# MikeIvanichev/norma

Measured on AMD Instinct MI355X. Metric: audio-sec/wall-sec (xRT) distil-large-v3 fp16 b32, higher is better.
Workload: dtype f16

## Files before the change

### norma_amd/csrc/k_attn_enc.hip

```cpp
#include "nh_kernels.h"

#ifndef ENC_ATTN_KERNEL
#define ENC_ATTN_KERNEL enc_attn_kernel
#define ENC_ATTN_LAUNCH launch_enc_attention
#endif
#define KT 64
#define QW 32
#ifndef ENC_ATTN_WAVES
#define ENC_ATTN_WAVES 8
#endif
#define QB (QW * ENC_ATTN_WAVES)
#define NTHR (64 * ENC_ATTN_WAVES)
#define NSLOT (NTHR >= 512 ? 1 : 512 / NTHR)
#define TILE_B 8192

__device__ __forceinline__ int swap23(int x) { return (x & ~12) | ((x & 4) << 1) | ((x & 8) >> 1); }

#ifndef ENC_ATTN_MINWAVES
#ifdef ENC_ATTN_PIPE
#define ENC_ATTN_MINWAVES 2
#else
#define ENC_ATTN_MINWAVES 4
#endif
#endif
__global__ __launch_bounds__(NTHR, (NTHR <= 512 ? ENC_ATTN_MINWAVES : 1)) void ENC_ATTN_KERNEL(const half_t *__restrict__ q, const half_t *__restrict__ k,
                                                         long ld, const half_t *__restrict__ vt,
                                                         half_t *__restrict__ out, long ldo, int S, int H) {
    __shared__ __attribute__((aligned(16))) char smem[2 * 2 * TILE_B];
    const int tid = threadIdx.x, lane = tid & 63, w = tid >> 6;
    const int r = lane & 31, hh = lane >> 5;
    const int b = blockIdx.z, h = blockIdx.y;
    const int q0 = blockIdx.x * QB + w * QW;
    const int nT = (S + KT - 1) / KT;

    half8 qf[4];
    {
        int qrow = q0 + r; if (qrow >= S) qrow = S - 1;
        const half_t *qp = q + ((long)b * S + qrow) * ld + h * NH_DH + 8 * hh;
#pragma unroll
        for (int ks = 0; ks < 4; ks++) qf[ks] = *reinterpret_cast<const half8 *>(qp + 16 * ks);
    }
    const half_t *kg[NSLOT]; const half_t *vg[NSLOT];
    int krow_off[NSLOT];
#pragma unroll
    for (int i = 0; i < NSLOT; i++) {
        int row = (tid >> 3) + (NTHR / 8) * i;
        int c = (tid & 7) ^ ((row >> 1) & 7);
        krow_off[i] = swap23(row);
        kg[i] = k + (long)b * S * ld + h * NH_DH + c * 8;
        vg[i] = vt + ((long)(b * H + h) * NH_DH + row) * NH_SP + c * 8;
    }
    u32x4 rk[NSLOT], rv[NSLOT];
    const bool stager = NTHR <= 512 || tid < 512;
    auto load_k = [&](int t) {
        if (!stager) return;
#pragma unroll
        for (int i = 0; i < NSLOT; i++) {
            int key = t * KT + krow_off[i]; if (key >= S) key = S - 1;
            rk[i] = *reinterpret_cast<const u32x4 *>(kg[i] + (long)key * ld);
        }
    };
    auto load_v = [&](int t) {
        if (!stager) return;
#pragma unroll
        for (int i = 0; i < NSLOT; i++) rv[i] = *reinterpret_cast<const u32x4 *>(vg[i] + t * KT);
    };
    auto store_k = [&](int buf) {
        if (!stager) return;
        u32x4 *lk = reinterpret_cast<u32x4 *>(smem + buf * 2 * TILE_B);
#pragma unroll
        for (int i = 0; i < NSLOT; i++) lk[tid + NTHR * i] = rk[i];
    };
    auto store_v = [&](int buf) {
        if (!stager) return;
        u32x4 *lv = reinterpret_cast<u32x4 *>(smem + buf * 2 * TILE_B + TILE_B);
#pragma unroll
        for (int i = 0; i < NSLOT; i++) lv[tid + NTHR * i] = rv[i];
    };
    auto load_tile = [&](int t) { load_k(t); load_v(t); };
    auto store_tile = [&](int buf) { store_k(buf); store_v(buf); };
    load_tile(0);
    store_tile(0);
#ifdef ENC_ATTN_PIPE
    if (nT > 1) { load_k(1); store_k(1); }
#endif
    __syncthreads();

    const int g = (r >> 1) & 7;
    const int offK0 = r * 128 + ((hh ^ g) << 4);
    const int offV0 = r * 128 + ((hh ^ g) << 4);

    f32x16 o0, o1;
#pragma unroll
    for (int i = 0; i < 16; i++) { o0[i] = 0.f; o1[i] = 0.f; }
    const f32x16 zero = {0.f, 0.f, 0.f, 0.f, 0.f, 0.f, 0.f, 0.f, 0.f, 0.f, 0.f, 0.f, 0.f, 0.f, 0.f, 0.f};
    const half_t one_h = hh == 0 ? (half_t)1.0f : (half_t)0.0f;
    const half8 kx = {one_h, one_h, (half_t)0.f, (half_t)0.f, (half_t)0.f, (half_t)0.f, (half_t)0.f, (half_t)0.f};
    half8 qx = {(half_t)0.f, (half_t)0.f, (half_t)0.f, (half_t)0.f, (half_t)0.f, (half_t)0.f, (half_t)0.f, (half_t)0.f};
    float m_ref = 0.f, l_run = 0.f;
    const float REBASE = 8.0f;

    f32x16 s0, s1;
    auto qk_phase = [&](const char *tk, f32x16 &s0, f32x16 &s1) {
        {
            half8 k0 = *reinterpret_cast<const half8 *>(tk + offK0);
            half8 k1 = *reinterpret_cast<const half8 *>(tk + 4096 + offK0);
            s0 = __builtin_amdgcn_mfma_f32_32x32x16_f16(k0, qf[0], zero, 0, 0, 0);
            s1 = __builtin_amdgcn_mfma_f32_32x32x16_f16(k1, qf[0], zero, 0, 0, 0);
        }
#pragma unroll
        for (int ks = 1; ks < 4; ks++) {
            half8 k0 = *reinterpret_cast<const half8 *>(tk + (offK0 ^ (ks << 5)));
            half8 k1 = *reinterpret_cast<const half8 *>(tk + 4096 + (offK0 ^ (ks << 5)));
            s0 = __builtin_amdgcn_mfma_f32_32x32x16_f16(k0, qf[ks], s0, 0, 0, 0);
            s1 = __builtin_amdgcn_mfma_f32_32x32x16_f16(k1, qf[ks], s1, 0, 0, 0);
        }
        s0 = __builtin_amdgcn_mfma_f32_32x32x16_f16(kx, qx, s0, 0, 0, 0);
        s1 = __builtin_amdgcn_mfma_f32_32x32x16_f16(kx, qx, s1, 0, 0, 0);
    };
    auto sm_head = [&](int t) {
        if (t * KT + KT > S) {
#pragma unroll
            for (int i = 0; i < 16; i++) {
                int rho = (i & 3) + 8 * (i >> 2) + 4 * hh;
                int key0 = t * KT + swap23(rho), key1 = t * KT + 32 + swap23(rho);
                if (key0 >= S) s0[i] = -INFINITY;
                if (key1 >= S) s1[i] = -INFINITY;
            }
        }
        float mx = fmaxf(fmaxf(s0[0], s0[1]), s0[2]);
#pragma unroll
        for (int i = 3; i < 15; i += 2) mx = fmaxf(fmaxf(mx, s0[i]), s0[i + 1]);
        mx = fmaxf(fmaxf(mx, s0[15]), s1[0]);
#pragma unroll
        for (int i = 1; i < 15; i += 2) mx = fmaxf(fmaxf(mx, s1[i]), s1[i + 1]);
        mx = fmaxf(mx, s1[15]);
        mx = fmaxf(mx, __shfl_xor(mx, 32));
        const bool reb = (t == 0) || (mx > REBASE);
        if (__builtin_amdgcn_ballot_w64(reb) != 0) {
            const float dlt = reb ? mx : 0.f;
            const float alpha = __builtin_amdgcn_exp2f(-dlt);
#pragma unroll
            for (int i = 0; i < 16; i++) { o0[i] *= alpha; o1[i] *= alpha; s0[i] -= dlt; s1[i] -= dlt; }
            l_run *= alpha;
            m_ref += dlt;
            const float nm = fminf(fmaxf(-m_ref, -60000.f), 60000.f);
            const half_t hi = (half_t)nm;
            const half_t lo = (half_t)(nm - (float)hi);
            qx[0] = hh == 0 ? hi : (half_t)0.f;
            qx[1] = hh == 0 ? lo : (half_t)0.f;
        }
    };
    auto sm_body = [&](const char *tv) {
        float ps = 0.f;
#pragma unroll
        for (int i = 0; i < 16; i++) {
            s0[i] = __builtin_amdgcn_exp2f(s0[i]); s1[i] = __builtin_amdgcn_exp2f(s1[i]);
            ps += s0[i]; ps += s1[i];
        }
        l_run += ps;
        half8 p00, p01, p10, p11;
#pragma unroll
        for (int j = 0; j < 8; j++) {
            p00[j] = (half_t)s0[j]; p01[j] = (half_t)s0[8 + j];
            p10[j] = (half_t)s1[j]; p11[j] = (half_t)s1[8 + j];
        }
        {
            half8 v;
            v = *reinterpret_cast<const half8 *>(tv + (offV0 ^ (0 << 4)));          o0 = __builtin_amdgcn_mfma_f32_32x32x16_f16(v, p00, o0, 0, 0, 0);
            v = *reinterpret_cast<const half8 *>(tv + 4096 + (offV0 ^ (0 << 4)));   o1 = __builtin_amdgcn_mfma_f32_32x32x16_f16(v, p00, o1, 0, 0, 0);
            v = *reinterpret_cast<const half8 *>(tv + (offV0 ^ (2 << 4)));          o0 = __builtin_amdgcn_mfma_f32_32x32x16_f16(v, p01, o0, 0, 0, 0);
            v = *reinterpret_cast<const half8 *>(tv + 4096 + (offV0 ^ (2 << 4)));   o1 = __builtin_amdgcn_mfma_f32_32x32x16_f16(v, p01, o1, 0, 0, 0);
            v = *reinterpret_cast<const half8 *>(tv + (offV0 ^ (4 << 4)));          o0 = __builtin_amdgcn_mfma_f32_32x32x16_f16(v, p10, o0, 0, 0, 0);
            v = *reinterpret_cast<const half8 *>(tv + 4096 + (offV0 ^ (4 << 4)));   o1 = __builtin_amdgcn_mfma_f32_32x32x16_f16(v, p10, o1, 0, 0, 0);
            v = *reinterpret_cast<const half8 *>(tv + (offV0 ^ (6 << 4)));          o0 = __builtin_amdgcn_mfma_f32_32x32x16_f16(v, p11, o0, 0, 0, 0);
            v = *reinterpret_cast<const half8 *>(tv + 4096 + (offV0 ^ (6 << 4)));   o1 = __builtin_amdgcn_mfma_f32_32x32x16_f16(v, p11, o1, 0, 0, 0);
        }
    };
#ifndef ENC_ATTN_PIPE
    int cur = 0;
    for (int t = 0; t < nT; t++) {
        const bool more = (t + 1 < nT);
        if (more) load_tile(t + 1);
        qk_phase(smem + cur * 2 * TILE_B, s0, s1);
        sm_head(t);
        sm_body(smem + cur * 2 * TILE_B + TILE_B);
        if (more) store_tile(cur ^ 1);
        __syncthreads();
        cur ^= 1;
    }
#else
    f32x16 n0, n1;
    qk_phase(smem, s0, s1);
    for (int t = 0; t < nT; t++) {
        if (t + 2 < nT) load_k(t + 2);
        if (t + 1 < nT) load_v(t + 1);
        sm_head(t);
        qk_phase(smem + ((t + 1) & 1) * 2 * TILE_B, n0, n1);
        sm_body(smem + (t & 1) * 2 * TILE_B + TILE_B);
#pragma unroll
        for (int i = 0; i < 18; i++) {
            __builtin_amdgcn_sched_group_barrier(0x008, 1, 0);
            __builtin_amdgcn_sched_group_barrier(0x002, ENC_ATTN_PIPE, 0);
        }
        if (t + 2 < nT) store_k(t & 1);
        if (t + 1 < nT) store_v((t + 1) & 1);
        __syncthreads();
        s0 = n0; s1 = n1;
    }
#endif
    const float l_tot = l_run + __shfl_xor(l_run, 32);
    const float inv = 1.0f / l_tot;
    const int qrow = q0 + r;
    if (qrow < S) {
        half_t *op = out + ((long)b * S + qrow) * ldo + h * NH_DH + 4 * hh;
#pragma unroll
        for (int gq = 0; gq < 4; gq++) {
            half4 a = {(half_t)(o0[4 * gq] * inv), (half_t)(o0[4 * gq + 1] * inv), (half_t)(o0[4 * gq + 2] * inv),
                       (half_t)(o0[4 * gq + 3] * inv)};
            half4 c = {(half_t)(o1[4 * gq] * inv), (half_t)(o1[4 * gq + 1] * inv), (half_t)(o1[4 * gq + 2] * inv),
                       (half_t)(o1[4 * gq + 3] * inv)};
            *reinterpret_cast<half4 *>(op + 8 * gq) = a;
            *reinterpret_cast<half4 *>(op + 32 + 8 * gq) = c;
        }
    }
}

void ENC_ATTN_LAUNCH(const half_t *q, const half_t *k, long ld, const half_t *vt, half_t *out, long ldo,
                          int B, int S, int H, hipStream_t st) {
    dim3 grid((S + QB - 1) / QB, H, B);
    hipLaunchKernelGGL(ENC_ATTN_KERNEL, grid, dim3(NTHR), 0, st, q, k, ld, vt, out, ldo, S, H);
}
```

Measured before the change: 6780.

## Stage encoder attention K/V tiles directly into LDS with a multi-buffer ring and XCD-aware order

Replaces the register-staged double buffer (global load to registers, then store to LDS) with direct global_load_lds DMA into a ring of 3 tile buffers. Synchronisation now uses explicit vmcnt waits and a raw s_barrier. The change also linearises the grid and remaps blocks so all query blocks of a (batch, head) pair land on the same XCD, for better L2 reuse of K/V, and it skips compute for waves whose queries fall past S. This is meant to hide global latency and cut VGPR and LDS-store traffic. In exchange it uses more LDS (48 KiB) and hand-tuned wait counts that must match the number of loads exactly.

```diff
diff --git a/norma_amd/csrc/enc_attn_order.h b/norma_amd/csrc/enc_attn_order.h
--- /dev/null
+++ b/norma_amd/csrc/enc_attn_order.h
@@ -0,0 +1,30 @@
+#pragma once
+
+#if defined(__HIPCC__) || defined(__CUDACC__)
+#define ENC_ATTN_ORDER_FN __host__ __device__ inline
+#else
+#define ENC_ATTN_ORDER_FN inline
+#endif
+
+#define ENC_ATTN_XCDS 8
+
+struct EncAttnSlot {
+    int pair;
+    int block;
+};
+
+ENC_ATTN_ORDER_FN int enc_attn_grid(int pairs, int nqb) {
+    return ENC_ATTN_XCDS * ((pairs + ENC_ATTN_XCDS - 1) / ENC_ATTN_XCDS) * nqb;
+}
+
+ENC_ATTN_ORDER_FN EncAttnSlot enc_attn_order(int i, int pairs, int nqb) {
+    const int xcd = i & (ENC_ATTN_XCDS - 1), slot = i / ENC_ATTN_XCDS;
+    const int q = pairs / ENC_ATTN_XCDS, r = pairs % ENC_ATTN_XCDS;
+    const int lp = slot / nqb;
+    const int count = q + (xcd < r ? 1 : 0);
+    const int first = xcd < r ? xcd * (q + 1) : r * (q + 1) + (xcd - r) * q;
+    EncAttnSlot s;
+    s.pair = lp < count ? first + lp : -1;
+    s.block = slot - lp * nqb;
+    return s;
+}
diff --git a/norma_amd/csrc/k_attn_enc.hip b/norma_amd/csrc/k_attn_enc.hip
--- a/norma_amd/csrc/k_attn_enc.hip
+++ b/norma_amd/csrc/k_attn_enc.hip
@@ -1,4 +1,5 @@
 #include "nh_kernels.h"
+#include "enc_attn_order.h"
 
 #ifndef ENC_ATTN_KERNEL
 #define ENC_ATTN_KERNEL enc_attn_kernel
@@ -6,32 +7,38 @@
 #endif
 #define KT 64
 #define QW 32
-#ifndef ENC_ATTN_WAVES
 #define ENC_ATTN_WAVES 8
-#endif
 #define QB (QW * ENC_ATTN_WAVES)
 #define NTHR (64 * ENC_ATTN_WAVES)
-#define NSLOT (NTHR >= 512 ? 1 : 512 / NTHR)
 #define TILE_B 8192
+#ifndef ENC_ATTN_RING
+#define ENC_ATTN_RING 3
+#endif
+static_assert(ENC_ATTN_RING >= 2 && ENC_ATTN_RING <= 4, "ring of 2 .. 4 tiles: <= 64 KiB of LDS, two workgroups per CU");
+
+typedef __attribute__((address_space(3))) void lds_void;
+typedef const __attribute__((address_space(1))) void gbl_void;
 
 __device__ __forceinline__ int swap23(int x) { return (x & ~12) | ((x & 4) << 1) | ((x & 8) >> 1); }
 
-#ifndef ENC_ATTN_MINWAVES
-#ifdef ENC_ATTN_PIPE
-#define ENC_ATTN_MINWAVES 2
-#else
-#define ENC_ATTN_MINWAVES 4
-#endif
-#endif
-__global__ __launch_bounds__(NTHR, (NTHR <= 512 ? ENC_ATTN_MINWAVES : 1)) void ENC_ATTN_KERNEL(const half_t *__restrict__ q, const half_t *__restrict__ k,
+__device__ __forceinline__ void wait_tiles_in_flight(int n) {
+    if (n >= 2) asm volatile("s_waitcnt vmcnt(4)" ::: "memory");
+    else if (n == 1) asm volatile("s_waitcnt vmcnt(2)" ::: "memory");
+    else asm volatile("s_waitcnt vmcnt(0)" ::: "memory");
+}
+
+__global__ __launch_bounds__(NTHR, 4) void ENC_ATTN_KERNEL(const half_t *__restrict__ q, const half_t *__restrict__ k,
                                                          long ld, const half_t *__restrict__ vt,
-                                                         half_t *__restrict__ out, long ldo, int S, int H) {
-    __shared__ __attribute__((aligned(16))) char smem[2 * 2 * TILE_B];
-    const int tid = threadIdx.x, lane = tid & 63, w = tid >> 6;
+                                                         half_t *__restrict__ out, long ldo, int S, int H, int pairs, int nqb) {
+    __shared__ __attribute__((aligned(16))) char smem[ENC_ATTN_RING * 2 * TILE_B];
+    const EncAttnSlot slot = enc_attn_order(blockIdx.x, pairs, nqb);
+    if (slot.pair < 0) return;
+    const int tid = threadIdx.x, lane = tid & 63, w = __builtin_amdgcn_readfirstlane(tid >> 6);
     const int r = lane & 31, hh = lane >> 5;
-    const int b = blockIdx.z, h = blockIdx.y;
-    const int q0 = blockIdx.x * QB + w * QW;
+    const int b = slot.pair / H, h = slot.pair - b * H;
+    const int q0 = slot.block * QB + w * QW;
     const int nT = (S + KT - 1) / KT;
+    const bool live = q0 < S;
 
     half8 qf[4];
     {
@@ -40,51 +47,31 @@
 #pragma unroll
         for (int ks = 0; ks < 4; ks++) qf[ks] = *reinterpret_cast<const half8 *>(qp + 16 * ks);
     }
-    const half_t *kg[NSLOT]; const half_t *vg[NSLOT];
-    int krow_off[NSLOT];
-#pragma unroll
-    for (int i = 0; i < NSLOT; i++) {
-        int row = (tid >> 3) + (NTHR / 8) * i;
-        int c = (tid & 7) ^ ((row >> 1) & 7);
-        krow_off[i] = swap23(row);
-        kg[i] = k + (long)b * S * ld + h * NH_DH + c * 8;
-        vg[i] = vt + ((long)(b * H + h) * NH_DH + row) * NH_SP + c * 8;
-    }
-    u32x4 rk[NSLOT], rv[NSLOT];
-    const bool stager = NTHR <= 512 || tid < 512;
-    auto load_k = [&](int t) {
-        if (!stager) return;
-#pragma unroll
-        for (int i = 0; i < NSLOT; i++) {
-            int key = t * KT + krow_off[i]; if (key >= S) key = S - 1;
-            rk[i] = *reinterpret_cast<const u32x4 *>(kg[i] + (long)key * ld);
-        }
-    };
-    auto load_v = [&](int t) {
-        if (!stager) return;
-#pragma unroll
-        for (int i = 0; i < NSLOT; i++) rv[i] = *reinterpret_cast<const u32x4 *>(vg[i] + t * KT);
-    };
-    auto store_k = [&](int buf) {
-        if (!stager) return;
-        u32x4 *lk = reinterpret_cast<u32x4 *>(smem + buf * 2 * TILE_B);
-#pragma unroll
-        for (int i = 0; i < NSLOT; i++) lk[tid + NTHR * i] = rk[i];
-    };
-    auto store_v = [&](int buf) {
-        if (!stager) return;
-        u32x4 *lv = reinterpret_cast<u32x4 *>(smem + buf * 2 * TILE_B + TILE_B);
-#pragma unroll
-        for (int i = 0; i < NSLOT; i++) lv[tid + NTHR * i] = rv[i];
-    };
-    auto load_tile = [&](int t) { load_k(t); load_v(t); };
-    auto store_tile = [&](int buf) { store_k(buf); store_v(buf); };
-    load_tile(0);
-    store_tile(0);
-#ifdef ENC_ATTN_PIPE
-    if (nT > 1) { load_k(1); store_k(1); }
-#endif
-    __syncthreads();
+    const int srow = tid >> 3;
+    const int krow_off = swap23(srow);
+    const int sc = (tid & 7) ^ ((srow >> 1) & 7);
+    const half_t *const kg = k + (long)b * S * ld + h * NH_DH + sc * 8;
+    const half_t *const vg = vt + ((long)(b * H + h) * NH_DH + srow) * NH_SP + sc * 8;
+    char *const wbase = smem + w * 1024;
+    const half_t *const kg0 = kg + (long)krow_off * ld;
+    auto stage = [&](int t, int buf) __attribute__((always_inline)) {
+        const half_t *ksrc;
+        if (t * KT + KT <= S) {
+            ksrc = kg0 + (long)t * KT * ld;
+        } else {
+            int key = t * KT + krow_off; if (key >= S) key = S - 1;
+            ksrc = kg + (long)key * ld;
+        }
+        __builtin_amdgcn_global_load_lds((gbl_void *)ksrc, (lds_void *)(wbase + buf * 2 * TILE_B), 16, 0, 0);
+        __builtin_amdgcn_global_load_lds((gbl_void *)(vg + t * KT), (lds_void *)(wbase + buf * 2 * TILE_B + TILE_B), 16, 0, 0);
+    };
+#pragma unroll
+    for (int u = 0; u < ENC_ATTN_RING - 1; u++)
+        if (u < nT) stage(u, u);
+    wait_tiles_in_flight(min(ENC_ATTN_RING - 2, nT - 1));
+    asm volatile("" : "+v"(qf[0]), "+v"(qf[1]), "+v"(qf[2]), "+v"(qf[3]));
+    __builtin_amdgcn_s_barrier();
+    __builtin_amdgcn_sched_barrier(0);
 
     const int g = (r >> 1) & 7;
     const int offK0 = r * 128 + ((hh ^ g) << 4);
@@ -177,38 +164,23 @@
             v = *reinterpret_cast<const half8 *>(tv + 4096 + (offV0 ^ (6 << 4)));   o1 = __builtin_amdgcn_mfma_f32_32x32x16_f16(v, p11, o1, 0, 0, 0);
         }
     };
-#ifndef ENC_ATTN_PIPE
-    int cur = 0;
-    for (int t = 0; t < nT; t++) {
-        const bool more = (t + 1 < nT);
-        if (more) load_tile(t + 1);
-        qk_phase(smem + cur * 2 * TILE_B, s0, s1);
-        sm_head(t);
-        sm_body(smem + cur * 2 * TILE_B + TILE_B);
-        if (more) store_tile(cur ^ 1);
-        __syncthreads();
-        cur ^= 1;
+    auto step = [&](int t, int buf) __attribute__((always_inline)) {
+        if (t + ENC_ATTN_RING - 1 < nT) stage(t + ENC_ATTN_RING - 1, (buf + ENC_ATTN_RING - 1) % ENC_ATTN_RING);
+        if (live) {
+            qk_phase(smem + buf * 2 * TILE_B, s0, s1);
+            sm_head(t);
+            sm_body(smem + buf * 2 * TILE_B + TILE_B);
+        }
+        __builtin_amdgcn_sched_barrier(0);
+        if (t + 1 < nT) wait_tiles_in_flight(min(ENC_ATTN_RING - 2, nT - 2 - t));
+        __builtin_amdgcn_s_barrier();
+        __builtin_amdgcn_sched_barrier(0);
+    };
+    for (int t = 0; t < nT; t += ENC_ATTN_RING) {
+#pragma unroll
+        for (int u = 0; u < ENC_ATTN_RING; u++)
+            if (t + u < nT) step(t + u, u);
     }
-#else
-    f32x16 n0, n1;
-    qk_phase(smem, s0, s1);
-    for (int t = 0; t < nT; t++) {
-        if (t + 2 < nT) load_k(t + 2);
-        if (t + 1 < nT) load_v(t + 1);
-        sm_head(t);
-        qk_phase(smem + ((t + 1) & 1) * 2 * TILE_B, n0, n1);
-        sm_body(smem + (t & 1) * 2 * TILE_B + TILE_B);
-#pragma unroll
-        for (int i = 0; i < 18; i++) {
-            __builtin_amdgcn_sched_group_barrier(0x008, 1, 0);
-            __builtin_amdgcn_sched_group_barrier(0x002, ENC_ATTN_PIPE, 0);
-        }
-        if (t + 2 < nT) store_k(t & 1);
-        if (t + 1 < nT) store_v((t + 1) & 1);
-        __syncthreads();
-        s0 = n0; s1 = n1;
-    }
-#endif
     const float l_tot = l_run + __shfl_xor(l_run, 32);
     const float inv = 1.0f / l_tot;
     const int qrow = q0 + r;
@@ -228,6 +200,6 @@
 
 void ENC_ATTN_LAUNCH(const half_t *q, const half_t *k, long ld, const half_t *vt, half_t *out, long ldo,
                           int B, int S, int H, hipStream_t st) {
-    dim3 grid((S + QB - 1) / QB, H, B);
-    hipLaunchKernelGGL(ENC_ATTN_KERNEL, grid, dim3(NTHR), 0, st, q, k, ld, vt, out, ldo, S, H);
+    const int pairs = B * H, nqb = (S + QB - 1) / QB;
+    hipLaunchKernelGGL(ENC_ATTN_KERNEL, dim3(enc_attn_grid(pairs, nqb)), dim3(NTHR), 0, st, q, k, ld, vt, out, ldo, S, H, pairs, nqb);
 }
```

After: 6809, median of 6. About the same (+0.4%).
